# mirsadm/motioncam-decoder

Measured on AMD Instinct MI355X. Metric: MPixels/s unpacked + achieved HBM GB/s %peak, 4K 12-bit, 1/2/4/8 GPUs, higher is better.
Workload: dtype u16; 1 GPU; 3840x2160 12-bit type-7 x 240 frames/GPU, Nat (smooth field + noise sigma 12); frames_per_gpu=240, width=3840, height=2160, bits=12, encoding=7, streams=1

## Files before the change

### motioncam_decoder_amd/build.py

```python
import os
import shutil
import subprocess
import sys

PKG = os.path.dirname(os.path.abspath(__file__))
ROOT = os.path.dirname(PKG)
LIB = os.path.join(PKG, "lib")
CSRC = os.path.join(PKG, "csrc")
SYNTH = os.path.join(PKG, "synth")
HOST = os.path.join(PKG, "host")

HIPCC = os.environ.get("HIPCC") or shutil.which("hipcc") or "/opt/rocm/bin/hipcc"
ARCH = "gfx950"


def _newer(target, sources):
    if not os.path.exists(target):
        return True
    t = os.path.getmtime(target)
    return any(os.path.getmtime(s) > t for s in sources)


def _run(cmd):
    print("+", " ".join(cmd), flush=True)
    subprocess.run(cmd, check=True)


HIP_SOURCES = ("mcraw_abi.hip", "mcraw_submit.hip", "mcraw_tune.hip", "mcraw_device.hip", "mcraw_hostmem.hip", "mcraw_pool.hip",
               "mcraw_type7.hip", "mcraw_type6.hip", "mcraw_encode7.hip", "mcraw_rgb.hip", "mcraw_shade.hip")
HIP_HEADERS = ("mcraw_plan.h", "mcraw_dev.h", "mcraw_host.h", "mcraw_race.h")
HIP_FLAGS = ["--offload-arch=" + ARCH, "-O3", "-std=c++17", "-fPIC", "-fno-gpu-rdc"]


def hip_sources():
    return [os.path.join(CSRC, f) for f in HIP_SOURCES]


def _objects(flags=(), tag="", force=False, only=None):
    obj = os.path.join(LIB, "obj")
    os.makedirs(obj, exist_ok=True)
    hdrs = [os.path.join(CSRC, f) for f in HIP_HEADERS] + [os.path.join(ROOT, "include", "mcraw_hip.h")]
    objs, jobs = [], []
    for src in hip_sources():
        if only is not None and src not in only:
            continue
        o = os.path.join(obj, os.path.basename(src)[:-4] + tag + ".o")
        objs.append(o)
        if force or _newer(o, [src] + hdrs):
            cmd = [HIPCC] + HIP_FLAGS + ["-Wall", "-Wno-unused-function"] + list(flags) + ["-c", "-o", o, src]
            print("+", " ".join(cmd), flush=True)
            jobs.append((subprocess.Popen(cmd), cmd))
    for pr, cmd in jobs:
        if pr.wait() != 0:
            raise subprocess.CalledProcessError(pr.returncode, cmd)
    return objs, bool(jobs)


def _link(out, objs):
    _run([HIPCC, "--offload-arch=" + ARCH, "-shared", "-fPIC", "-fno-gpu-rdc", "-o", out] + objs + ["-lpthread"])


def build_variant(out, flags=()):
    import hashlib
    import re
    os.makedirs(os.path.dirname(os.path.abspath(out)), exist_ok=True)
    names = [re.sub(r"^-D([A-Za-z0-9_]+).*$", r"\1", f) for f in flags if f.startswith("-D")]
    everything = len(names) != len(flags) or any(n in open(os.path.join(CSRC, h)).read() for n in names for h in HIP_HEADERS)
    touched = [s for s in hip_sources() if everything or any(n in open(s).read() for n in names)]
    tag = ".v" + hashlib.sha1(" ".join(flags).encode()).hexdigest()[:10]
    plain, _ = _objects(only=[s for s in hip_sources() if s not in touched])
    special, _ = _objects(flags, tag, only=touched)
    _link(out, plain + special)
    return out


TEST_VARIANTS = (["-DMCRAW_FORCE_SEGW"], ["-DMCRAW_INJECT_MUTE7"], ["-DMCRAW_INJECT_LOST"])


def prebuild_test_variants():
    import tempfile
    with tempfile.TemporaryDirectory() as d:
        for i, flags in enumerate(TEST_VARIANTS):
            build_variant(os.path.join(d, "v%d.so" % i), flags)


def build_hip(force=False):
    os.makedirs(LIB, exist_ok=True)
    out = os.path.join(LIB, "libmcraw_hip.so")
    if os.environ.get("MCRAW_DIAG"):
        objs, built = _objects(["-DMCRAW_DIAG"], ".diag", force)
    else:
        objs, built = _objects(force=force)
    if force or built or _newer(out, objs):
        _link(out, objs)
    return out


def build_timeline(force=False):
    out = os.path.join(LIB, "timeline", "libmcraw_hip.so")
    if force or _newer(out, hip_sources() + [os.path.join(CSRC, f) for f in HIP_HEADERS]):
        build_variant(out, ["-Wall", "-Wno-unused-function", "-DMCRAW_TIMELINE"])
    return out


def build_synth(force=False):
    out = os.path.join(SYNTH, "libmcraw_synth.so")
    src = os.path.join(SYNTH, "mcraw_synth.c")
    if force or _newer(out, [src]):
        _run(["gcc", "-O3", "-march=x86-64-v3", "-fPIC", "-std=c11", "-Wall", "-Wextra", "-shared", "-o", out, src, "-lm"])
    return out


def build_host(force=False):
    os.makedirs(LIB, exist_ok=True)
    out = os.path.join(LIB, "libmotioncam_decoder.so")
    srcs = [os.path.join(HOST, f) for f in ("Decoder.cpp", "RawData.cpp", "Writer.cpp")]
    if not all(os.path.exists(s) for s in srcs):
        return None
    hdrs = [os.path.join(HOST, "include", "motioncam", f) for f in ("Decoder.hpp", "Container.hpp", "RawData.hpp", "Writer.hpp",
                                                                     "mcraw_container.h")]
    hdrs.append(os.path.join(HOST, "WorkerPool.hpp"))
    inc = ["-I" + os.path.join(HOST, "include"), "-I" + os.path.join(HOST, "thirdparty"), "-I" + os.path.join(ROOT, "include")]
    if force or _newer(out, srcs + hdrs):
        _run(["g++", "-O2", "-std=c++17", "-fPIC", "-shared", "-Wall"] + inc + ["-o", out] + srcs +
             ["-L" + LIB, "-lmcraw_hip", "-lpthread", "-Wl,-rpath,$ORIGIN"])
    tool = os.path.join(LIB, "mcraw_export")
    tsrc = os.path.join(HOST, "mcraw_export.cpp")
    if os.path.exists(tsrc) and (force or _newer(tool, [tsrc, out])):
        _run(["g++", "-O2", "-std=c++17", "-Wall"] + inc + ["-o", tool, tsrc, "-L" + LIB, "-lmotioncam_decoder",
             "-lmcraw_hip", "-lpthread", "-Wl,-rpath,$ORIGIN"])
    return out


def build_all(force=False, targets=("hip", "synth", "host")):
    res = {}
    if "hip" in targets:
        res["hip"] = build_hip(force)
    if "synth" in targets:
        res["synth"] = build_synth(force)
    if "host" in targets:
        res["host"] = build_host(force)
    return res


if __name__ == "__main__":
    if len(sys.argv) > 2 and sys.argv[1] == "variant":
        build_variant(sys.argv[2], sys.argv[3:])
        sys.exit(0)
    args = [a for a in sys.argv[1:] if not a.startswith("-")]
    build_all(force="--force" in sys.argv, targets=tuple(args) or ("hip", "synth", "host"))
```

### motioncam_decoder_amd/csrc/mcraw_type7.hip

```cpp
#include <algorithm>
#include <cstdlib>

#include "mcraw_dev.h"

#include "../../include/mcraw_hip.h"

namespace mcraw {

#define TM(p, s, n, l) ((uint32_t)((p) * 8) | ((uint32_t)(s) << 8) | ((uint32_t)((1u << (n)) - 1u) << 16) | ((uint32_t)(l) << 24))
#define Z 0u
#define ROW1(k) {TM(0, k, 1, 0), Z, Z, Z}
#define ROW2(k) {TM((k) >> 2, 2 * ((k)&3), 2, 0), Z, Z, Z}
#define ROW4(k) {TM((k) >> 1, 4 * ((k)&1), 4, 0), Z, Z, Z}
#define ROW8(k) {TM(k, 0, 8, 0), Z, Z, Z}
#define ROW10(k) {TM(5 * ((k) >> 2) + ((k)&3), 0, 8, 0), Z, Z, TM(5 * ((k) >> 2) + 4, 2 * ((k)&3), 2, 0)}
__constant__ uint32_t c_tab7[9 * 8][4] = {
    {Z, Z, Z, Z}, {Z, Z, Z, Z}, {Z, Z, Z, Z}, {Z, Z, Z, Z}, {Z, Z, Z, Z}, {Z, Z, Z, Z}, {Z, Z, Z, Z}, {Z, Z, Z, Z},
    ROW1(0), ROW1(1), ROW1(2), ROW1(3), ROW1(4), ROW1(5), ROW1(6), ROW1(7),
    ROW2(0), ROW2(1), ROW2(2), ROW2(3), ROW2(4), ROW2(5), ROW2(6), ROW2(7),
    {TM(0, 0, 3, 0), Z, Z, Z}, {TM(0, 3, 3, 0), Z, Z, Z}, {TM(0, 6, 2, 0), TM(2, 6, 1, 2), Z, Z},
    {TM(1, 0, 3, 0), Z, Z, Z}, {TM(1, 3, 3, 0), Z, Z, Z}, {TM(1, 6, 2, 0), TM(2, 7, 1, 2), Z, Z},
    {TM(2, 0, 3, 0), Z, Z, Z}, {TM(2, 3, 3, 0), Z, Z, Z},
    ROW4(0), ROW4(1), ROW4(2), ROW4(3), ROW4(4), ROW4(5), ROW4(6), ROW4(7),
    {TM(0, 0, 5, 0), Z, Z, Z}, {TM(1, 0, 5, 0), Z, Z, Z}, {TM(2, 0, 5, 0), Z, Z, Z}, {TM(3, 0, 5, 0), Z, Z, Z},
    {TM(4, 0, 5, 0), Z, Z, Z}, {TM(0, 5, 3, 0), TM(3, 5, 2, 3), Z, Z}, {TM(1, 5, 3, 0), TM(4, 5, 2, 3), Z, Z},
    {TM(2, 5, 3, 0), TM(3, 7, 1, 3), TM(4, 7, 1, 4), Z},
    {TM(0, 0, 6, 0), Z, Z, Z}, {TM(1, 0, 6, 0), Z, Z, Z}, {TM(2, 0, 6, 0), Z, Z, Z}, {TM(3, 0, 6, 0), Z, Z, Z},
    {TM(4, 0, 6, 0), Z, Z, Z}, {TM(5, 0, 6, 0), Z, Z, Z},
    {TM(0, 6, 2, 0), TM(1, 6, 2, 2), TM(2, 6, 2, 4), Z}, {TM(3, 6, 2, 0), TM(4, 6, 2, 2), TM(5, 6, 2, 4), Z},
    ROW8(0), ROW8(1), ROW8(2), ROW8(3), ROW8(4), ROW8(5), ROW8(6), ROW8(7),
    ROW10(0), ROW10(1), ROW10(2), ROW10(3), ROW10(4), ROW10(5), ROW10(6), ROW10(7),
};
#undef TM
#undef Z

__device__ __forceinline__ uint32_t term_off(uint32_t t) { return t & 0xffu; }
__device__ __forceinline__ uint32_t term_shr(uint32_t t) { return (t >> 8) & 31u; }
__device__ __forceinline__ uint32_t term_mask(uint32_t t) { return __builtin_amdgcn_perm(t, t, 0x02020202u); }
__device__ __forceinline__ uint32_t term_shl(uint32_t t) { return (t >> 24) & 31u; }

struct Unpacked { uint32_t x[4]; };

template <bool ALIGNED8>
__device__ __forceinline__ uint2 lds_read8(const uint8_t *__restrict__ base, uint32_t off)
{
    if (ALIGNED8)
        return *reinterpret_cast<const uint2 *>(base + off);
    const uint32_t *w = reinterpret_cast<const uint32_t *>(base) + (off >> 2);
    const uint32_t sh = (off & 3u) * 8u;
    const uint32_t w0 = w[0], w1 = w[1], w2 = w[2];
    return make_uint2(__builtin_amdgcn_alignbit(w1, w0, sh), __builtin_amdgcn_alignbit(w2, w1, sh));
}

template <bool ALIGNED8>
__device__ __forceinline__ Unpacked unpack8(const uint8_t *__restrict__ base, uint32_t blk, uint32_t cidx, uint32_t k,
                                            const uint4 *__restrict__ s_tab)
{
    Unpacked u;
    if (cidx >= 9u) {
        const uint2 a = lds_read8<ALIGNED8>(base, blk + 16u * k);
        const uint2 b = lds_read8<ALIGNED8>(base, blk + 16u * k + 8u);
        u.x[0] = a.x; u.x[1] = a.y; u.x[2] = b.x; u.x[3] = b.y;
        return u;
    }
    const uint4 row = s_tab[cidx * 8u + k];
    uint32_t lo = 0, hi = 0;
    const uint32_t tms[3] = {row.x, row.y, row.z};
#pragma unroll
    for (int t = 0; t < 3; t++) {
        const uint32_t tm = tms[t];
        if (!ALIGNED8 && t > 0 && !__any(tm != 0u))
            continue;
        const uint2 p = lds_read8<ALIGNED8>(base, blk + term_off(tm));
        const uint32_t m = term_mask(tm);
        lo |= ((p.x >> term_shr(tm)) & m) << term_shl(tm);
        hi |= ((p.y >> term_shr(tm)) & m) << term_shl(tm);
    }
    const uint32_t th = row.w;
    uint32_t lo8 = 0, hi8 = 0;
    if (ALIGNED8 || __any(th != 0u)) {
        const uint2 ph = lds_read8<ALIGNED8>(base, blk + term_off(th));
        const uint32_t mh = term_mask(th);
        lo8 = (ph.x >> term_shr(th)) & mh;
        hi8 = (ph.y >> term_shr(th)) & mh;
    }
    u.x[0] = __builtin_amdgcn_perm(lo8, lo, 0x05010400u);
    u.x[1] = __builtin_amdgcn_perm(lo8, lo, 0x07030602u);
    u.x[2] = __builtin_amdgcn_perm(hi8, hi, 0x05010400u);
    u.x[3] = __builtin_amdgcn_perm(hi8, hi, 0x07030602u);
    return u;
}

#ifndef MCRAW_SIDE_T
#define MCRAW_SIDE_T 512
#endif
#ifndef MCRAW_SIDE_LPT
#define MCRAW_SIDE_LPT 4
#endif
#ifndef MCRAW_SIDE_LCAP
#define MCRAW_SIDE_LCAP 512
#endif
#ifndef MCRAW_SPEC_WARM
#define MCRAW_SPEC_WARM 8192
#endif
constexpr uint32_t SIDE_XL = 9;
constexpr uint32_t SIDE_OUT = 0xFFu;
constexpr uint32_t SIDE_DEAD = 0xFEu;
static_assert(ITEM_SPLIT == 2, "k7_side sums the block lengths of half a record per item");

template <int PATTERN>
__device__ __forceinline__ uint32_t swz_xor(uint32_t v)
{
    return static_cast<uint32_t>(__builtin_amdgcn_ds_swizzle(static_cast<int>(v), PATTERN));
}

__device__ __forceinline__ void lds_barrier()
{
    asm volatile("s_waitcnt lgkmcnt(0)\n\ts_barrier" ::: "memory");
}

__device__ __forceinline__ uint2 side_strides(const uint4 v, uint32_t odd)
{
    const uint32_t pick = odd ? 0x07050301u : 0x06040200u;
    uint32_t st[2];
#pragma unroll
    for (int i = 0; i < 2; i++) {
        const uint32_t h4 = i ? __builtin_amdgcn_perm(v.w, v.z, pick) : __builtin_amdgcn_perm(v.y, v.x, pick);
        const uint32_t hb = (h4 >> 4) & 0x0F0F0F0Fu;
        const uint32_t sel = hb & 0x07070707u;
        const uint32_t lo = __builtin_amdgcn_perm(0x08060504u, 0x03020100u, sel);
        const uint32_t hi = __builtin_amdgcn_perm(0x10101010u, 0x100A0A08u, sel);
        const uint32_t g = (hb >> 3) & 0x01010101u;
        const uint32_t m = byte_mask(g);
        st[i] = (((hi & m) | (lo & ~m)) << 2) + 0x01010101u;
    }
    return make_uint2(st[0], st[1]);
}

#ifdef MCRAW_DIAG
#ifndef SIDE_PROF_BLOCK
#define SIDE_PROF_BLOCK 1u
#endif
__device__ unsigned long long g_side_prof[2][256];
#define SIDE_STAMP(slot)                                                                                               \
    do {                                                                                                               \
        if (blockIdx.x == SIDE_PROF_BLOCK && (tid == 0u || tid == 64u) && tl_n_ < 255u) {                              \
            const unsigned long long now_ = __builtin_amdgcn_s_memtime();                                              \
            g_side_prof[tid ? 1 : 0][++tl_n_] = (static_cast<unsigned long long>(slot) << 48) | (now_ - stamp_);       \
            g_side_prof[tid ? 1 : 0][0] = tl_n_;                                                                        \
        }                                                                                                              \
    } while (0)
#else
#define SIDE_STAMP(slot)
#endif

template <uint32_t SIDE_T, uint32_t SIDE_LPT, uint32_t SIDE_LCAP, uint32_t SPEC_WARM, bool PARTS, bool LASTC>
__global__ __launch_bounds__(SIDE_T) __attribute__((amdgpu_waves_per_eu(4, 4))) void k7_side(const Work7 W)
{
    constexpr uint32_t SIDE_PIECE = 16 * SIDE_T * SIDE_LPT;
    constexpr uint32_t SIDE_HALF = SIDE_PIECE / 2;
    constexpr uint32_t SIDE_BYTES = SIDE_PIECE + SIDE_XL * 16 + 16;
    __shared__ __attribute__((aligned(16))) uint8_t s_b[SIDE_BYTES];
    __shared__ __attribute__((aligned(16))) uint8_t s_T[SIDE_HALF + 80];
    __shared__ __attribute__((aligned(16))) uint16_t s_L[2][SIDE_LCAP];
    __shared__ __attribute__((aligned(16))) uint16_t s_len[2][2 * SIDE_LCAP];
    __shared__ uint4 s_tab[72];
    __shared__ __attribute__((aligned(16))) uint32_t s_st[2][4];
    __shared__ uint2 s_seg[64];
    __shared__ int32_t s_err;

    const uint32_t nfr = static_cast<uint32_t>(W.n7), nsb = PARTS ? W.nsplit[0] : 1u, nsr = PARTS ? W.nsplit[1] : 1u;
    const uint32_t bq = blockIdx.x / nfr, f = blockIdx.x - bq * nfr;
    const uint32_t s = bq < nsr ? 1u : 0u, part = s ? bq : bq - nsr, nsp = s ? nsr : nsb;
    const uint32_t fs = (nsb + nsr) * f + (s ? nsb : 0u) + part;
    const uint32_t tid = threadIdx.x, lane = tid & 63u;
    const uint32_t wave = __builtin_amdgcn_readfirstlane(tid >> 6);
#ifdef MCRAW_DIAG
    const unsigned long long stamp_ = __builtin_amdgcn_s_memtime();
    uint32_t tl_n_ = 0, nsteps_ = 0;
#endif
    if (tid < 72u)
        s_tab[tid] = reinterpret_cast<const uint4 *>(c_tab7)[tid];
    if (tid < 80u)
        s_T[SIDE_HALF + tid] = static_cast<uint8_t>(SIDE_OUT);
    if (tid == 0u)
        s_err = 0;

    const Plan7 PL = W.plans[f];
    const Plan7 *P = &PL;
    int32_t *status = W.status + fs;
    const uint32_t len = P->len;
    const __amdgpu_buffer_rsrc_t rs = frame_rsrc(P->in, len);
    SIDE_STAMP(10);

    const uint4 hv = ld_b128(rs, 0);
    const uint32_t encW = __builtin_amdgcn_readfirstlane(hv.x), encH = __builtin_amdgcn_readfirstlane(hv.y);
    const uint32_t bitsOff = __builtin_amdgcn_readfirstlane(hv.z), refsOff = __builtin_amdgcn_readfirstlane(hv.w);
    const uint32_t so = s ? refsOff : bitsOff;
    const uint64_t A0 = (static_cast<uint64_t>(so) + 4u) & ~15ull;
    const uint32_t odd = (so + 4u) & 1u;
    struct Lines {
        uint4 v[SIDE_LPT], x;
    };
    auto load_piece = [&](Lines &r, uint32_t piece) {
        const uint64_t base = A0 + static_cast<uint64_t>(piece) * SIDE_PIECE;
#pragma unroll
        for (uint32_t j = 0; j < SIDE_LPT; j++) {
            const uint64_t o = base + 16ull * (tid + SIDE_T * j);
            r.v[j] = o < len ? ld_b128(rs, static_cast<uint32_t>(o)) : make_uint4(0, 0, 0, 0);
        }
        r.x = make_uint4(0, 0, 0, 0);
        if (tid < SIDE_XL) {
            const uint64_t o = base + 16ull * (SIDE_T * SIDE_LPT + tid);
            r.x = o < len ? ld_b128(rs, static_cast<uint32_t>(o)) : make_uint4(0, 0, 0, 0);
        }
    };
    Lines nx, ny;
    load_piece(nx, 0u);
    int32_t err = 0;
    uint32_t tilesX = 0, nblk = 0, R = 0;
    if (len < 16u || bitsOff > len || refsOff > len || (encW & 63u) != 0u || encW < static_cast<uint32_t>(P->width) ||
        encW == 0u || encH == 0u || (encH & 3u) != 0u ||
        static_cast<uint64_t>(encW) * encH >= (1ull << 31)) {
        err = MCRAW_E_HEADER;
    } else {
        tilesX = encW >> 6;
        nblk = 4u * tilesX * (encH >> 2);
        R = (nblk + GROUP_BLOCKS - 1u) / GROUP_BLOCKS;
        if (R > P->ngroups)
            err = E_GEOMETRY;
        else if (so + 4u > len || so + 4u < so)
            err = MCRAW_E_TRUNCATED;
        else {
            const uint32_t count = ld_u8(rs, so) | (ld_u8(rs, so + 1u) << 8) | (ld_u8(rs, so + 2u) << 16) |
                                   (ld_u8(rs, so + 3u) << 24);
            if (__builtin_amdgcn_readfirstlane(count) < nblk)
                err = MCRAW_E_SIDESTREAM;
        }
    }
    SIDE_STAMP(11);
    Frame7 *const FR = W.frames + f;
    if (s == 0u && part == 0u && tid == 0u) {
        FR->in = P->in;
        FR->out = P->out;
        FR->len = len;
        FR->width = P->width;
        FR->rows = min(static_cast<uint32_t>(P->height), encH);
        FR->tilesX = tilesX;
        FR->nblk = err ? 0u : nblk;
        FR->fast_store = P->fast_store;
        FR->encH = encH;
        FR->pstride = P->pstride;
        for (uint32_t q = err ? 0u : nsb - 1u; q < 3u; q++) {
            FR->part_item[q] = 0xFFFFFFFFu;
            FR->part_len[q] = 0u;
        }
        W.status[W.nstatus + f] = static_cast<int32_t>(encH);
    }
    if (err) {
        if (tid == 0u)
            *status = err;
        return;
    }
    constexpr uint32_t ENDX_ = 0xFFFFFFFFu;
    uint32_t m_lo = 0u, m_hi = 0xFFFFFFFFu, np_guess = 0xFFFFFFFFu;
    if (nsp > 1u) {
        const uint32_t other = s ? bitsOff : refsOff;
        const uint64_t end_guess = other > so ? other : len;
        const uint64_t npieces = (end_guess - A0 + SIDE_PIECE - 1u) / SIDE_PIECE;
        np_guess = static_cast<uint32_t>(npieces);
        m_lo = static_cast<uint32_t>(part * npieces / nsp);
        if (part + 1u < nsp)
            m_hi = static_cast<uint32_t>((part + 1u) * npieces / nsp);
    }
    uint64_t *const sync = W.sync + (static_cast<size_t>(2u * f + s) * MAX_SPLIT7 + part) * 2u;
    uint16_t *const rp_base = (PARTS && nsp > 1u && W.rpos) ? W.rpos + (static_cast<size_t>(2u * f + s) * MAX_SPLIT7 + part) * W.Rmax : nullptr;
    const __amdgpu_buffer_rsrc_t rsp = frame_rsrc(reinterpret_cast<const uint8_t *>(rp_base), rp_base ? 2u * W.Rmax : 0u);
    uint32_t rleft = 0u, rnext = 0u, rexit = ENDX_;
    bool rdead = false;
    constexpr uint32_t ENDX = ENDX_;

    uint8_t *bits = W.bits + static_cast<size_t>(f) * W.Rmax * 64u;
    uint16_t *refs = W.refs + static_cast<size_t>(f) * W.Rmax * 64u;
    uint32_t *goff = W.grp_off + static_cast<size_t>(f) * (W.Rmax * ITEM_SPLIT + 1u);

    uint32_t upc = 0;
    uint32_t bb = 0;
    uint32_t tb = 0;
    uint32_t n = 0;
    uint64_t carry = 0u;
    uint32_t n_first = 0xFFFFFFFFu;
    int32_t lane_err = 0;
    bool dead = false;
    uint32_t decode_from = 0u;
    constexpr uint32_t NOENTRY = 0xFFFFFFFEu;
    static_assert(SPEC_WARM <= SIDE_HALF, "a speculative count starts inside the piece in front of the part's first");

    auto store_bytes = [&](const Lines &r) {
#pragma unroll
        for (uint32_t j = 0; j < SIDE_LPT; j++)
            reinterpret_cast<uint4 *>(s_b)[tid + SIDE_T * j] = r.v[j];
        if (tid < SIDE_XL)
            reinterpret_cast<uint4 *>(s_b)[SIDE_T * SIDE_LPT + tid] = r.x;
    };
    auto build_strides = [&](const Lines &r, uint32_t piece) {
        const uint64_t base = A0 + static_cast<uint64_t>(piece) * SIDE_PIECE;
        const uint64_t left = len - min(static_cast<uint64_t>(len), base);
        const uint32_t lim = static_cast<uint32_t>(min(left, static_cast<uint64_t>(1u << 30)));
#pragma unroll
        for (uint32_t j = 0; j < SIDE_LPT; j++) {
            const uint32_t line = tid + SIDE_T * j;
            uint2 st = side_strides(r.v[j], odd);
            if (16u * line + 16u + 130u > lim) {
                uint32_t w[2] = {st.x, st.y};
#pragma unroll
                for (uint32_t i = 0; i < 8u; i++) {
                    const uint32_t sv = (w[i >> 2] >> (8u * (i & 3u))) & 0xffu;
                    if (16u * line + 2u * i + odd + 2u * sv > lim)
                        w[i >> 2] = (w[i >> 2] & ~(0xffu << (8u * (i & 3u)))) | (SIDE_DEAD << (8u * (i & 3u)));
                }
                st = make_uint2(w[0], w[1]);
            }
            reinterpret_cast<uint2 *>(s_T)[line] = st;
        }
    };
    #ifndef MCRAW_SEGW_RATIO
#define MCRAW_SEGW_RATIO 3u
#endif
#ifndef MCRAW_WARM_SEGS
#define MCRAW_WARM_SEGS 4
#endif
    constexpr uint32_t SEG_C = SIDE_HALF / 64u, WARM_C = MCRAW_WARM_SEGS * SEG_C, SEG_NONE = 0x7FFFu, SEG_DEADX = 0xFFFFu;
#ifdef MCRAW_FORCE_SEGW
    bool segw = true, seg_valid = false;
#else
    bool segw = false, seg_valid = false;
#endif
    uint32_t seg_total = 0, seg_done = 0, seg_exit = 0;
    auto seg_chain = [&](bool on, uint32_t pos, uint32_t segs, uint32_t sege, uint32_t &ent, uint32_t &cnt, uint32_t &ex) {
        pos = on ? pos : SIDE_HALF;
        sege = on ? sege : 0u;
        bool stop;
        do {
#pragma unroll
            for (int u = 0; u < 2; u++) {
                const uint32_t code = s_T[pos];
                stop = pos >= sege || code >= SIDE_DEAD;
                const bool inseg = !stop && pos >= segs;
                ent = min(ent, inseg ? pos : SEG_NONE);
                cnt += inseg ? 1u : 0u;
                pos += stop ? 0u : code;
            }
#ifdef MCRAW_DIAG
            nsteps_ += 2;
#endif
        } while (__any(!stop));
        if (on)
            ex = pos >= sege ? pos : SEG_DEADX;
    };
    auto seg_walk = [&](uint32_t org) {
        const uint32_t segs = org + lane * SEG_C;
        const bool act = segs < SIDE_HALF;
        const uint32_t sege = min(segs + SEG_C, SIDE_HALF);
        const bool on_chain = lane < WARM_C / SEG_C;
        uint32_t ent = SEG_NONE, cnt = 0, ex = SEG_DEADX;
        seg_chain(act, on_chain ? org : segs - WARM_C, segs, sege, ent, cnt, ex);
        uint32_t src = SEG_NONE;
        for (uint32_t round = 0; round < 64u; round++) {
            const uint32_t want = wave_prev(ex, ex);
            const uint32_t claim = src != SEG_NONE ? src : ent != SEG_NONE ? ent : ex;
            const bool bad = act && !on_chain && claim != want;
            if (__ballot(bad) == 0ull)
                break;
            if (bad) {
                ent = SEG_NONE;
                cnt = 0;
                ex = SEG_DEADX;
                src = want;
            }
            seg_chain(bad && want != SEG_DEADX, want, segs, sege, ent, cnt, ex);
        }
        uint32_t total;
        const uint32_t off = wave_excl_scan(act ? cnt : 0u, lane, &total);
        s_seg[lane] = make_uint2((ent & 0xFFFFu) | (cnt << 16), off);
        const uint32_t nact = (SIDE_HALF - org + SEG_C - 1u) / SEG_C;
        seg_exit = static_cast<uint32_t>(__builtin_amdgcn_readlane(static_cast<int>(ex), static_cast<int>(min(nact, 64u) - 1u)));
        seg_total = total;
        seg_done = 0;
        seg_valid = true;
    };
    auto seg_list = [&](uint16_t *L, uint32_t take) {
        const uint2 sv = s_seg[lane];
        const uint32_t cnt = sv.x >> 16, off = sv.y, lo = seg_done, hi = seg_done + take;
        uint32_t pos = sv.x & 0xFFFFu, kk = off;
        const uint32_t kend = min(off + cnt, hi);
        bool part = cnt != 0u && off < hi && off + cnt > lo;
        pos = part ? pos : SIDE_HALF;
        while (__any(part)) {
            const uint32_t code = s_T[pos];
            if (part && kk >= lo)
                L[kk - lo] = static_cast<uint16_t>(pos);
            kk++;
            part = part && kk < kend;
            pos = part ? pos + code : SIDE_HALF;
        }
    };
    auto walk = [&](uint32_t lst, uint32_t pu, uint32_t SU, uint32_t room, bool fresh) {
        uint16_t *L = s_L[lst];
        uint32_t cnt = 0, why = 2u;
        if (!segw && pu < SIDE_HALF) {
            uint32_t nb, take, nxt, passes = 0;
            bool go;
            do {
                const uint32_t u = pu + lane * SU;
                const uint32_t code = s_T[min(u, SIDE_HALF)];
                const unsigned long long m = __ballot(code != SU);
                nb = m == 0ull ? 64u : static_cast<uint32_t>(__builtin_ctzll(m));
                take = min(nb, room - cnt);
                if (lane < take)
                    L[cnt + lane] = static_cast<uint16_t>(u);
                nxt = static_cast<uint32_t>(__builtin_amdgcn_readlane(static_cast<int>(code), static_cast<int>(nb & 63u)));
                cnt += take;
                pu += take * SU;
                go = take == nb && cnt < room && (nb == 64u || nxt < SIDE_DEAD);
                SU = (go && nb != 64u) ? nxt : SU;
                passes++;
                segw = go && passes >= 8u && passes * MCRAW_SEGW_RATIO > cnt;
#ifdef MCRAW_DIAG
                nsteps_++;
#endif
            } while (go && !segw);
            if (segw) {
            } else if (take < nb) {
                why = 1u;
            } else if (cnt >= room) {
                why = 1u;
                SU = (nb != 64u && nxt < SIDE_DEAD) ? nxt : 0u;
            } else {
                why = nxt == SIDE_OUT ? 2u : 3u;
                SU = 0u;
            }
            if (segw)
                seg_valid = false;
        } else if (!segw) {
            SU = 0u;
        }
        if (segw && pu < SIDE_HALF) {
            if (fresh || !seg_valid)
                seg_walk(pu);
            const uint32_t take = min(room - cnt, seg_total - seg_done);
            if (take)
                seg_list(L + cnt, take);
            seg_done += take;
            cnt += take;
            SU = 0u;
            if (seg_done == seg_total) {
                why = seg_exit == SEG_DEADX ? 3u : 2u;
                pu = seg_exit == SEG_DEADX ? 0u : seg_exit;
                seg_valid = false;
            } else {
                why = 1u;
                pu = 0u;
            }
        } else if (segw) {
            SU = 0u;
        }
        if (lane == 0u)
            *reinterpret_cast<uint4 *>(s_st[lst]) = make_uint4(pu, cnt, why, SU);
    };

    const uint32_t k = lane & 7u, sub = lane >> 3;
    const uint32_t first_cand = static_cast<uint32_t>((so + 4u) & 15u) >> 1;
    static_assert((2u * SIDE_LCAP) % 512u == 0u, "whole passes of 512 items");
    auto scan_unit = [&](uint32_t par, uint32_t n0, uint32_t cnt) {
        const uint32_t nitems = 2u * cnt;
        for (uint32_t base = 0; base < nitems; base += 512u) {
            const uint32_t i0 = base + 8u * lane;
            uint4 lv = make_uint4(0u, 0u, 0u, 0u);
            if (i0 < nitems)
                lv = *reinterpret_cast<const uint4 *>(&s_len[par][i0]);
            uint32_t a[8] = {lv.x & 0xffffu, lv.x >> 16, lv.y & 0xffffu, lv.y >> 16,
                             lv.z & 0xffffu, lv.z >> 16, lv.w & 0xffffu, lv.w >> 16};
            uint32_t mine = 0;
#pragma unroll
            for (uint32_t i = 0; i < 8u; i++) {
                a[i] = i0 + i < nitems ? a[i] : 0u;
                mine += a[i];
            }
            uint32_t utot;
            const uint32_t ex = wave_excl_scan(mine, lane, &utot);
            uint32_t o = static_cast<uint32_t>(carry) + ex;
#pragma unroll
            for (uint32_t i = 0; i < 8u; i++) {
                if (i0 + i < nitems)
                    goff[2u * n0 + i0 + i] = o;
                o += a[i];
            }
            carry += utot;
        }
    };

#ifdef MCRAW_INJECT_MUTE7
    constexpr uint32_t SPIN7 = 1u << 6;
#else
    constexpr uint32_t SPIN7 = 1u << 19;
#endif
    __shared__ uint32_t s_ask[4];
    bool told = part + 1u >= nsp;
    auto tell = [&](uint32_t count, uint32_t where) {
        if (!told && tid == 0u) {
#ifdef MCRAW_INJECT_MUTE7
            if (part != 0u)
#endif
            {
                look_put(sync, W.epoch, count);
                look_put(sync + 1, W.epoch, where);
            }
        }
        told = true;
    };
    auto ask = [&](uint32_t &count, uint32_t &where) {
        lds_barrier();
        if (tid == 0u) {
            uint32_t c = 0u, w = first_cand, ok = 1u;
            if (part) {
                ok = 0u;
                for (uint32_t spin = 0; spin < SPIN7; spin++) {
                    if (look_get(sync - 2, W.epoch, &c) && look_get(sync - 1, W.epoch, &w)) {
                        ok = 1u;
                        break;
                    }
                    __builtin_amdgcn_s_sleep(8);
                }
            }
            s_ask[0] = c;
            s_ask[1] = w;
            s_ask[2] = ok;
        }
        lds_barrier();
        count = s_ask[0];
        where = s_ask[1];
        return s_ask[2] != 0u;
    };
    auto nothing_to_decode = [&]() {
        if (tid == 0u && s == 0u && nsp > 1u) {
            if (part + 1u < nsp)
                FR->part_len[part] = 0u;
            if (part)
                FR->part_item[part - 1u] = 0xFFFFFFFFu;
        }
    };

    uint32_t run_piece = 0u, run_cand = first_cand, run_n = 0u;
    uint32_t nx_piece = 0u;
    uint32_t exitc = ENDX;
    bool go = true;
    if (nsp > 1u) {
        const bool empty = m_lo >= m_hi, lastp = part + 1u >= nsp;
        const bool owns0 = !empty && m_lo == 0u;
        const uint32_t m_chi = lastp ? np_guess : m_hi;
        const bool lastc = LASTC && lastp && !owns0 && rp_base != nullptr && m_chi > m_lo && m_chi != 0xFFFFFFFFu;
        const bool spec = !empty && !owns0 && (!lastp || lastc);
        uint32_t entry = NOENTRY, cnt1 = 0u, exit1 = ENDX;
        bool dead1 = false;
        bool counted = false;
        if (!empty && (!lastp || lastc)) {
            counted = true;
            uint32_t spiece = 0xFFFFFFFFu;
            uint32_t cpiece = spec ? m_lo - 1u : 0u, lst = 0u;
            if (spec)
                load_piece(nx, cpiece);
            build_strides(nx, cpiece);
            load_piece(nx, cpiece + 1u);
            nx_piece = cpiece + 1u;
            lds_barrier();
            if (wave == 0u)
                walk(0u, spec ? SIDE_HALF - SPEC_WARM : first_cand, 0u, spec ? SIDE_LCAP : min(R, SIDE_LCAP), true);
            for (;;) {
                lds_barrier();
                const uint4 st4 = *reinterpret_cast<const uint4 *>(s_st[lst]);
                const uint32_t pu = __builtin_amdgcn_readfirstlane(st4.x);
                const uint32_t total = __builtin_amdgcn_readfirstlane(st4.y);
                const uint32_t why = __builtin_amdgcn_readfirstlane(st4.z);
                const uint32_t SU = __builtin_amdgcn_readfirstlane(st4.w);
                const uint32_t npc = why == 2u ? cpiece + 1u : cpiece;
                if (cpiece >= m_lo) {
                    if (rp_base && total) {
                        const uint16_t *Lc = s_L[lst];
                        for (uint32_t i = tid; i < total; i += SIDE_T)
                            if (cnt1 + i < W.Rmax)
                                rp_base[cnt1 + i] = static_cast<uint16_t>(Lc[i] | ((i == 0u && cpiece != spiece) ? 0x8000u : 0u));
                        spiece = cpiece;
                    }
                    cnt1 += total;
                    dead1 = dead1 || why == 3u;
                }
// ... 33 lines not shown
        uint32_t pn = 0u, pw = first_cand;
        const bool ok = owns0 ? true : ask(pn, pw);
        SIDE_STAMP(21);
        decode_from = m_lo;
        if (!ok) {
            if (empty) {
                decode_from = 0xFFFFFFFFu;
                if (m_hi == 0u) {
                    tell(0u, first_cand);
                    nothing_to_decode();
                    go = false;
                }
            }
        } else if (!owns0 && (pw == ENDX || pn >= R)) {
            tell(pn, ENDX);
            nothing_to_decode();
            go = false;
        } else if (empty) {
            tell(pn, pw);
            nothing_to_decode();
            go = false;
        } else if (lastp) {
            run_piece = m_lo, run_cand = owns0 ? first_cand : pw, run_n = pn;
            if (lastc && pw == entry)
                replay_from_count();
        } else if (owns0 || pw == entry) {
            const uint32_t upto = pn + cnt1;
            tell(min(upto, R), upto >= R || dead1 || exit1 == ENDX ? ENDX : exit1);
            run_piece = m_lo, run_cand = owns0 ? first_cand : entry, run_n = pn;
            replay_from_count();
        } else {
            run_piece = m_lo, run_cand = pw, run_n = pn;
        }
        if (go && run_n >= R) {
            tell(run_n, ENDX);
            nothing_to_decode();
            go = false;
        }
    }

    uint32_t cur = 0;
    uint32_t prev_n = 0, prev_total = 0;
    if (go) {
    lds_barrier();
    upc = bb = tb = run_piece;
    n = run_n;
#ifdef MCRAW_FORCE_SEGW
    segw = true;
#else
    segw = false;
#endif
    seg_valid = false;
    carry = run_piece == 0u && decode_from == 0u ? 16u : 0u;
    if (nx_piece != run_piece)
        load_piece(nx, run_piece);
    store_bytes(nx);
    SIDE_STAMP(12);
    if (!rleft)
        build_strides(nx, run_piece);
    load_piece(nx, run_piece + 1u);
    load_piece(ny, run_piece + 2u);
    uint4 rq = make_uint4(0u, 0u, 0u, 0u);
    auto rfetch = [&](uint32_t at) { rq = ld_b128_nt(rsp, 2u * (at + 8u * lane)); };
    auto replay = [&](uint32_t lst, uint32_t room) {
        const uint32_t n = min(room, rleft);
        const uint32_t w4[4] = {rq.x, rq.y, rq.z, rq.w};
        uint32_t mine = 8u, ment = 0u;
#pragma unroll
        for (int i = 7; i >= 0; i--) {
            const uint32_t idx = 8u * lane + static_cast<uint32_t>(i), e = (w4[i >> 1] >> (16 * (i & 1))) & 0xffffu;
            const bool hit = idx >= 1u && idx < n && (e & 0x8000u) != 0u;
            mine = hit ? static_cast<uint32_t>(i) : mine;
            ment = hit ? e : ment;
        }
        const unsigned long long m = __ballot(mine != 8u);
        uint32_t take = n, pu = 0u, why = 1u;
        if (m) {
            const uint32_t fl = static_cast<uint32_t>(__builtin_ctzll(m));
            take = 8u * fl + wave_lane(mine, fl);
            pu = SIDE_HALF + (wave_lane(ment, fl) & 0x7fffu);
            why = 2u;
        } else if (n == rleft) {
            if (rdead)
                why = 3u;
            else if (rexit != ENDX)
                why = 2u, pu = SIDE_HALF + rexit;
        }
        if (8u * lane < take)
            *reinterpret_cast<uint4 *>(&s_L[lst][8u * lane]) = make_uint4(rq.x & 0x7fff7fffu, rq.y & 0x7fff7fffu, rq.z & 0x7fff7fffu, rq.w & 0x7fff7fffu);
        if (lane == 0u)
            *reinterpret_cast<uint4 *>(s_st[lst]) = make_uint4(pu, take, why, 0u);
        rfetch(rnext + take);
    };
    lds_barrier();
    SIDE_STAMP(13);
    if (wave == 0u) {
        if (rleft) {
            rfetch(0u);
            replay(0u, min(R - run_n, SIDE_LCAP / 4u));
        } else
            walk(0u, run_cand, 0u, min(R - run_n, SIDE_LCAP / 4u), true);
    }
    SIDE_STAMP(14);
    while (true) {
        lds_barrier();
        SIDE_STAMP(0);
        const uint4 st4 = *reinterpret_cast<const uint4 *>(s_st[cur]);
        const uint32_t pu = __builtin_amdgcn_readfirstlane(st4.x);
        const uint32_t total = __builtin_amdgcn_readfirstlane(st4.y);
        const uint32_t why = __builtin_amdgcn_readfirstlane(st4.z);
        const uint32_t SU = __builtin_amdgcn_readfirstlane(st4.w);
        const uint32_t npc = why == 2u ? upc + 1u : upc;
        const bool last = n + total >= R || why == 3u || npc >= m_hi;
        const bool skip = upc < decode_from;
        if (!skip && n_first == 0xFFFFFFFFu)
            n_first = n;
        if (npc > upc && npc == m_hi)
            exitc = pu - SIDE_HALF;
        if (rleft) {
            rleft -= min(total, rleft);
            rnext += total;
        }
        const bool moved = upc > bb, build = !last && npc > tb && rleft == 0u;
        if (moved) {
            store_bytes(nx);
            bb = upc;
            nx = ny;
            load_piece(ny, bb + 2u);
        }
        if (build) {
            build_strides(nx, npc);
            tb = npc;
        }
        if (moved || build)
            lds_barrier();
        SIDE_STAMP(1);
        if (wave == 0u) {
            if (!last) {
                if (rleft)
                    replay(cur ^ 1u, min(R - (n + total), SIDE_LCAP));
                else
                    walk(cur ^ 1u, npc > upc ? pu - SIDE_HALF : pu, SU, min(R - (n + total), SIDE_LCAP), npc > upc);
            }
            SIDE_STAMP(2);
            if (s == 0u && prev_total)
                scan_unit(cur ^ 1u, prev_n, prev_total);
            SIDE_STAMP(5);
        } else if (!skip) {
            const uint8_t *B = s_b;
            const uint16_t *L = s_L[cur];
            constexpr uint32_t STEP = (SIDE_T / 64u - 1u) * 8u;
            uint32_t q = (wave - 1u) * 8u + sub;
            uint32_t ro_n = q < total ? 2u * L[q] + odd : 0u;
            uint32_t hd_n = *reinterpret_cast<const uint16_t *>(B + (ro_n & ~1u)) | (static_cast<uint32_t>(B[(ro_n & ~1u) + 2u]) << 16);
            for (uint32_t qb = (wave - 1u) * 8u; qb < total; qb += STEP, q += STEP) {
                const bool live = q < total;
                const uint32_t ro = ro_n;
                const uint32_t hd = hd_n >> (8u * (ro & 1u));
                ro_n = q + STEP < total ? 2u * L[q + STEP] + odd : 0u;
                hd_n = *reinterpret_cast<const uint16_t *>(B + (ro_n & ~1u)) | (static_cast<uint32_t>(B[(ro_n & ~1u) + 2u]) << 16);
                const uint32_t b0 = live ? hd & 0xffu : 0u, b1 = (hd >> 8) & 0xffu;
                const uint32_t hb = b0 >> 4, ref = ((b0 & 15u) << 8) | b1;
                Unpacked U = unpack8<false>(B, ro + 2u, cls7_of(hb), k, s_tab);
                const u16x2 rr = __builtin_bit_cast(u16x2, ref | (ref << 16));
#pragma unroll
                for (int i = 0; i < 4; i++)
                    U.x[i] = __builtin_bit_cast(uint32_t, __builtin_bit_cast(u16x2, U.x[i]) + rr);
                const uint32_t r = n + q;
                const uint32_t idx = r * 64u + 8u * k;
                if (s == 1u) {
                    if (live)
                        *reinterpret_cast<uint4 *>(refs + idx) = make_uint4(U.x[0], U.x[1], U.x[2], U.x[3]);
                    continue;
                }
                const uint32_t nvalid = live ? min(8u, nblk - min(nblk, idx)) : 0u;
                if (nvalid < 8u) {
#pragma unroll
                    for (uint32_t i = 0; i < 4u; i++)
                        U.x[i] &= nvalid >= 2u * i + 2u ? 0xffffffffu : nvalid == 2u * i + 1u ? 0xffffu : 0u;
                }
                uint32_t c[4], over = 0;
#pragma unroll
                for (uint32_t i = 0; i < 4u; i++) {
                    c[i] = __builtin_bit_cast(uint32_t, __builtin_elementwise_min(__builtin_bit_cast(u16x2, U.x[i]),
                                                                                  __builtin_bit_cast(u16x2, 0x00100010u)));
                    over |= c[i] ^ U.x[i];
                }
                if (over)
                    lane_err |= MCRAW_E_SIDESTREAM;
                const uint32_t bytes_lo = __builtin_amdgcn_perm(c[1], c[0], 0x06040200u);
                const uint32_t bytes_hi = __builtin_amdgcn_perm(c[3], c[2], 0x06040200u);
                if (live)
                    *reinterpret_cast<uint2 *>(bits + idx) = make_uint2(bytes_lo, bytes_hi);
                uint32_t l8 = 0;
#pragma unroll
                for (uint32_t i = 0; i < 2u; i++) {
                    const uint32_t v4 = i ? bytes_hi : bytes_lo;
                    const uint32_t sel = v4 & 0x07070707u;
                    const uint32_t lo = __builtin_amdgcn_perm(0x08060504u, 0x03020100u, sel);
                    const uint32_t hi = __builtin_amdgcn_perm(0x10101010u, 0x100A0A08u, sel);
                    const uint32_t g = (v4 >> 3) & 0x01010101u;
                    const uint32_t m = byte_mask(g);
                    const uint32_t l4 = ((hi & m) | (lo & ~m)) | (v4 & 0x10101010u);
                    l8 = __builtin_amdgcn_sad_u8(l4, 0u, l8);
                }
                l8 += swz_xor<0x041F>(l8);
                l8 += swz_xor<0x081F>(l8);
                if (live && (k & 3u) == 0u)
                    s_len[cur][2u * q + (k >> 2)] = static_cast<uint16_t>(l8 << 3);
            }
            SIDE_STAMP(3);
        }
        prev_n = n;
        prev_total = skip ? 0u : total;
        n += total;
        if (last) {
            dead = why == 3u && n < R && !skip;
            break;
        }
        upc = npc;
        cur ^= 1u;
    }
    tell(min(n, R), n >= R || dead || exitc == ENDX ? ENDX : exitc);
    if (s == 0u && prev_total) {
        lds_barrier();
        if (wave == 0u)
            scan_unit(cur, prev_n, prev_total);
    }
    if (tid == 0u) {
        if (dead)
            lane_err |= MCRAW_E_TRUNCATED;
        if (s == 0u) {
            const uint32_t c32 = static_cast<uint32_t>(min(carry, static_cast<uint64_t>(0xffffffffu)));
            if (n >= R && !dead && n_first != 0xFFFFFFFFu) {
                goff[ITEM_SPLIT * R] = c32;
                if (nsp == 1u && carry > len)
                    lane_err |= MCRAW_E_TRUNCATED;
            }
            if (nsp > 1u) {
                if (part + 1u < nsp)
                    FR->part_len[part] = n_first != 0xFFFFFFFFu ? c32 : 0u;
                if (part)
                    FR->part_item[part - 1u] = n_first != 0xFFFFFFFFu ? ITEM_SPLIT * n_first : 0xFFFFFFFFu;
            }
        }
    }
    }
    if (lane_err)
        atomicOr(&s_err, lane_err);
    lds_barrier();
    if (tid == 0u)
        *status = s_err;
    SIDE_STAMP(15);
#ifdef MCRAW_DIAG
    if (blockIdx.x == SIDE_PROF_BLOCK && tid == 0u)
        g_side_prof[0][255] = nsteps_;
#endif
}

constexpr int PAY_LDS = ITEM_SPAN + 16 + 32;
constexpr uint32_t PAY_CHUNKS = ITEM_SPAN / 16 + 1;

struct ItemS {
    uint32_t valid;
    uint32_t g, nblk, tilesX;
    uint32_t base16, n16, head;
    int32_t width, rows;
    uint32_t fast;
    const uint8_t *in;
    uint32_t len;
    uint16_t *out;
    size_t meta;
    uint32_t lean;
    uint32_t pstride;
};

__device__ __forceinline__ ItemS item_scalars(const Work7 &W, uint32_t item, uint32_t first_frame, uint32_t class_groups)
{
    ItemS I;
    const uint32_t per = W.Rmax * ITEM_SPLIT;
    const uint32_t cper = class_groups * ITEM_SPLIT;
    const uint32_t fc = item / cper;
    const uint32_t f = first_frame + fc;
    const uint32_t g = item - fc * cper;
    const Frame7 *F = W.frames + f;
    const uint32_t nblk = F->nblk;
    const uint32_t *grp = W.grp_off + static_cast<size_t>(f) * (per + 1u) + g;
    I.valid = g * ITEM_BLOCKS < nblk ? 1u : 0u;
    uint32_t start = 0, end = 0;
    if (I.valid) {
        start = grp[0];
        end = grp[1];
        if (W.nsplit[0] > 1u) {
            uint32_t ps = 0u, pe = 0u, sum_s = 0u;
            uint64_t e64 = end;
#pragma unroll
            for (uint32_t q = 0; q < 3u; q++) {
                const uint32_t pi = F->part_item[q];
                ps = g >= pi ? q + 1u : ps;
                pe = g + 1u >= pi && pi != 0xFFFFFFFFu ? q + 1u : pe;
            }
#pragma unroll
            for (uint32_t q = 0; q < 3u; q++) {
                const uint32_t pl = F->part_len[q];
                sum_s += q < ps ? pl : 0u;
                e64 += q < pe ? pl : 0u;
            }
            start += sum_s;
            end = static_cast<uint32_t>(e64);
            if ((g + 1u) * ITEM_BLOCKS >= nblk && e64 > F->len)
                atomicOr(W.status + (W.nsplit[0] + W.nsplit[1]) * f, MCRAW_E_TRUNCATED);
        }
    }
    I.g = g;
    I.nblk = nblk;
    I.tilesX = F->tilesX;
    I.base16 = start & ~15u;
    I.head = start - I.base16;
    I.n16 = I.valid ? min((end - min(end, I.base16) + 15u) >> 4, PAY_CHUNKS) : 0u;
    I.width = F->width;
    I.rows = static_cast<int32_t>(F->rows);
    I.fast = F->fast_store;
    I.in = F->in;
    I.len = F->len;
    I.out = F->out;
    I.meta = static_cast<size_t>(f) * W.Rmax * 64u + static_cast<size_t>(g) * ITEM_BLOCKS;
    I.lean = 0u;
    I.pstride = F->pstride;
    return I;
}

template <bool NT = false, int POST = 0>
__device__ __forceinline__ void store_px8(const ItemS &I, const Post &post, uint32_t y, uint32_t x, uint32_t p[4])
{
    const uint32_t width = static_cast<uint32_t>(I.width);
    if (y >= static_cast<uint32_t>(I.rows) || x >= width)
        return;
    if constexpr (POST >= PK_F32) {
        float_store8<NT, POST>(I.out, post, post.inv, width, I.pstride, y, x, p, min(8u, width - x), I.fast != 0u);
        return;
    } else if (POST) {
        post_store8<NT, POST>(I.out, post, width, y, x, p, min(8u, width - x), I.fast != 0u, POST != 16 && I.lean != 0u);
        return;
    }
    uint16_t *dst = I.out + static_cast<size_t>(y) * static_cast<size_t>(width) + x;
    if (I.fast && x + 8u <= width) {
        typedef uint32_t u32x4 __attribute__((ext_vector_type(4)));
        const u32x4 v = {p[0], p[1], p[2], p[3]};
        if (NT)
            store_stream16(dst, v);
        else
            *gptr<u32x4>(dst) = v;
    } else if (x + 8u <= width) {
        typedef uint32_t u32x4_u __attribute__((ext_vector_type(4), aligned(2)));
        const u32x4_u v = {p[0], p[1], p[2], p[3]};
        *gptr<u32x4_u>(dst) = v;
    } else {
        const uint32_t n = width - x;
#pragma unroll
        for (uint32_t i = 0; i < 8u; i++)
// ... 213 lines not shown
```

Before: 1.980 million MPixels/s.

## Add wave-uniform class fast paths to type-7 side decode and restructure run scan

In the side-stream decode loop, when all lanes of a wave share one block class, the code now uses specialised unpack routines per class. For small classes in the bit pass it computes the output bytes directly and skips the generic clamp and pack. The run-scan loop is reorganised into groups of four ballot steps with raised wave priority, the L index is prefetched two steps ahead, and the ds_swizzle reductions are replaced by DPP quad permutes. A compile flag keeps the old generic path as a test variant. The cost is extra branches, ballots and code size.

```diff
diff --git a/motioncam_decoder_amd/build.py b/motioncam_decoder_amd/build.py
--- a/motioncam_decoder_amd/build.py
+++ b/motioncam_decoder_amd/build.py
@@ -74,7 +74,7 @@
     return out
 
 
-TEST_VARIANTS = (["-DMCRAW_FORCE_SEGW"], ["-DMCRAW_INJECT_MUTE7"], ["-DMCRAW_INJECT_LOST"])
+TEST_VARIANTS = (["-DMCRAW_FORCE_SEGW"], ["-DMCRAW_INJECT_MUTE7"], ["-DMCRAW_INJECT_LOST"], ["-DMCRAW_SIDE_GENERIC"])
 
 
 def prebuild_test_variants():
diff --git a/motioncam_decoder_amd/csrc/mcraw_type7.hip b/motioncam_decoder_amd/csrc/mcraw_type7.hip
--- a/motioncam_decoder_amd/csrc/mcraw_type7.hip
+++ b/motioncam_decoder_amd/csrc/mcraw_type7.hip
@@ -91,6 +91,61 @@
     return u;
 }
 
+struct __attribute__((packed, aligned(1))) PackedU2 { uint32_t x, y; };
+__device__ __forceinline__ uint2 lds_read8_any(const uint8_t *__restrict__ base, uint32_t off)
+{
+#ifdef MCRAW_SIDE_READ64
+    const PackedU2 v = *reinterpret_cast<const PackedU2 *>(base + off);
+    return make_uint2(v.x, v.y);
+#else
+    return lds_read8<false>(base, off);
+#endif
+}
+
+template <uint32_t CLS>
+__device__ __forceinline__ uint2 side_bytes_class(const uint8_t *__restrict__ base, uint32_t blk, uint32_t k)
+{
+    static_assert(CLS == 1u || CLS == 2u || CLS == 4u || CLS == 7u, "classes of one term");
+    constexpr uint32_t LOG = CLS == 1u ? 0u : CLS == 2u ? 1u : CLS == 4u ? 2u : 3u, N = 1u << LOG;
+    constexpr uint32_t MASK = ((1u << N) - 1u) * 0x01010101u;
+    const uint2 p = lds_read8_any(base, blk + 8u * (k >> (3u - LOG)));
+    if (LOG == 3u)
+        return p;
+    const uint32_t sh = (k & ((8u >> LOG) - 1u)) << LOG;
+    return make_uint2((p.x >> sh) & MASK, (p.y >> sh) & MASK);
+}
+
+template <uint32_t CLS>
+__device__ __forceinline__ Unpacked side_unpack_class(const uint8_t *__restrict__ base, uint32_t blk, uint32_t k)
+{
+    Unpacked u;
+    if (CLS == 0u) {
+        u.x[0] = u.x[1] = u.x[2] = u.x[3] = 0u;
+        return u;
+    }
+    if (CLS == 9u) {
+        const uint2 a = lds_read8_any(base, blk + 16u * k);
+        const uint2 b = lds_read8_any(base, blk + 16u * k + 8u);
+        u.x[0] = a.x; u.x[1] = a.y; u.x[2] = b.x; u.x[3] = b.y;
+        return u;
+    }
+    uint2 lo, hi8 = make_uint2(0u, 0u);
+    if (CLS == 8u) {
+        const uint32_t g = 40u * (k >> 2);
+        lo = lds_read8_any(base, blk + g + 8u * (k & 3u));
+        const uint2 ph = lds_read8_any(base, blk + g + 32u);
+        const uint32_t sh = 2u * (k & 3u);
+        hi8 = make_uint2((ph.x >> sh) & 0x03030303u, (ph.y >> sh) & 0x03030303u);
+    } else {
+        lo = side_bytes_class<(CLS == 1u || CLS == 2u || CLS == 4u) ? CLS : 7u>(base, blk, k);
+    }
+    u.x[0] = __builtin_amdgcn_perm(hi8.x, lo.x, 0x05010400u);
+    u.x[1] = __builtin_amdgcn_perm(hi8.x, lo.x, 0x07030602u);
+    u.x[2] = __builtin_amdgcn_perm(hi8.y, lo.y, 0x05010400u);
+    u.x[3] = __builtin_amdgcn_perm(hi8.y, lo.y, 0x07030602u);
+    return u;
+}
+
 #ifndef MCRAW_SIDE_T
 #define MCRAW_SIDE_T 512
 #endif
@@ -108,10 +163,10 @@
 constexpr uint32_t SIDE_DEAD = 0xFEu;
 static_assert(ITEM_SPLIT == 2, "k7_side sums the block lengths of half a record per item");
 
-template <int PATTERN>
-__device__ __forceinline__ uint32_t swz_xor(uint32_t v)
-{
-    return static_cast<uint32_t>(__builtin_amdgcn_ds_swizzle(static_cast<int>(v), PATTERN));
+template <int CTRL>
+__device__ __forceinline__ uint32_t quad_perm(uint32_t v)
+{
+    return static_cast<uint32_t>(__builtin_amdgcn_update_dpp(0, static_cast<int>(v), CTRL, 0xf, 0xf, true));
 }
 
 __device__ __forceinline__ void lds_barrier()
@@ -409,39 +464,58 @@
         uint16_t *L = s_L[lst];
         uint32_t cnt = 0, why = 2u;
         if (!segw && pu < SIDE_HALF) {
-            uint32_t nb, take, nxt, passes = 0;
-            bool go;
-            do {
-                const uint32_t u = pu + lane * SU;
-                const uint32_t code = s_T[min(u, SIDE_HALF)];
-                const unsigned long long m = __ballot(code != SU);
-                nb = m == 0ull ? 64u : static_cast<uint32_t>(__builtin_ctzll(m));
-                take = min(nb, room - cnt);
-                if (lane < take)
-                    L[cnt + lane] = static_cast<uint16_t>(u);
-                nxt = static_cast<uint32_t>(__builtin_amdgcn_readlane(static_cast<int>(code), static_cast<int>(nb & 63u)));
-                cnt += take;
-                pu += take * SU;
-                go = take == nb && cnt < room && (nb == 64u || nxt < SIDE_DEAD);
-                SU = (go && nb != 64u) ? nxt : SU;
-                passes++;
-                segw = go && passes >= 8u && passes * MCRAW_SEGW_RATIO > cnt;
+            __builtin_amdgcn_s_setprio(3);
+            uint32_t nb, take, nxt, lim, left = room, passes = 0, SUp = SU;
+            for (;;) {
+                uint32_t i = 4u;
+                bool more;
+                do {
+                    const uint32_t u = __umul24(lane, SU) + pu;
+                    const uint32_t code = s_T[min(u, SIDE_HALF)];
+                    const unsigned long long m = __ballot(code != SU);
+                    nb = m == 0ull ? 64u : static_cast<uint32_t>(__builtin_ctzll(m));
+                    take = min(nb, left);
+                    if (lane < take)
+                        L[cnt + lane] = static_cast<uint16_t>(u);
+                    nxt = static_cast<uint32_t>(__builtin_amdgcn_readlane(static_cast<int>(code), static_cast<int>(nb & 63u)));
+                    cnt += take;
+                    pu += take * SU;
 #ifdef MCRAW_DIAG
-                nsteps_++;
-#endif
-            } while (go && !segw);
+                    nsteps_++;
+#endif
+                    lim = nxt < SIDE_DEAD ? left : 0u;
+                    asm volatile("" : "+s"(lim));
+                    i--;
+                    uint32_t lim4 = min(lim, i << 16);
+                    asm volatile("" : "+s"(lim4));
+                    more = nb < lim4;
+                    left -= take;
+                    SUp = SU;
+                    SU = nxt;
+                } while (more);
+                if (nb >= lim) {
+                    left += take;
+                    SU = SUp;
+                    break;
+                }
+                passes += 4u;
+                if (passes >= 8u && passes * MCRAW_SEGW_RATIO > cnt) {
+                    segw = true;
+                    break;
+                }
+            }
+            __builtin_amdgcn_s_setprio(0);
             if (segw) {
+                seg_valid = false;
             } else if (take < nb) {
                 why = 1u;
-            } else if (cnt >= room) {
+            } else if (take == left) {
                 why = 1u;
                 SU = (nb != 64u && nxt < SIDE_DEAD) ? nxt : 0u;
             } else {
                 why = nxt == SIDE_OUT ? 2u : 3u;
                 SU = 0u;
             }
-            if (segw)
-                seg_valid = false;
         } else if (!segw) {
             SU = 0u;
         }
@@ -781,44 +855,86 @@
             constexpr uint32_t STEP = (SIDE_T / 64u - 1u) * 8u;
             uint32_t q = (wave - 1u) * 8u + sub;
             uint32_t ro_n = q < total ? 2u * L[q] + odd : 0u;
+            uint32_t ro_nn = q + STEP < total ? 2u * L[q + STEP] + odd : 0u;
             uint32_t hd_n = *reinterpret_cast<const uint16_t *>(B + (ro_n & ~1u)) | (static_cast<uint32_t>(B[(ro_n & ~1u) + 2u]) << 16);
             for (uint32_t qb = (wave - 1u) * 8u; qb < total; qb += STEP, q += STEP) {
                 const bool live = q < total;
                 const uint32_t ro = ro_n;
                 const uint32_t hd = hd_n >> (8u * (ro & 1u));
-                ro_n = q + STEP < total ? 2u * L[q + STEP] + odd : 0u;
+                ro_n = ro_nn;
                 hd_n = *reinterpret_cast<const uint16_t *>(B + (ro_n & ~1u)) | (static_cast<uint32_t>(B[(ro_n & ~1u) + 2u]) << 16);
+                const uint32_t l_nn = L[min(q + 2u * STEP, SIDE_LCAP - 1u)];
                 const uint32_t b0 = live ? hd & 0xffu : 0u, b1 = (hd >> 8) & 0xffu;
                 const uint32_t hb = b0 >> 4, ref = ((b0 & 15u) << 8) | b1;
-                Unpacked U = unpack8<false>(B, ro + 2u, cls7_of(hb), k, s_tab);
-                const u16x2 rr = __builtin_bit_cast(u16x2, ref | (ref << 16));
-#pragma unroll
-                for (int i = 0; i < 4; i++)
-                    U.x[i] = __builtin_bit_cast(uint32_t, __builtin_bit_cast(u16x2, U.x[i]) + rr);
+                const uint32_t cls = cls7_of(hb);
                 const uint32_t r = n + q;
                 const uint32_t idx = r * 64u + 8u * k;
+                Unpacked U;
+                uint32_t bytes_lo = 0u, bytes_hi = 0u;
+                uint32_t path = 0u;
+#ifndef MCRAW_SIDE_GENERIC
+                if (qb + 8u <= total) {
+                    const uint32_t c0 = __builtin_amdgcn_readfirstlane(cls);
+                    if (__ballot(cls != c0) == 0ull) {
+                        if (s == 1u) {
+                            path = 1u;
+                            switch (c0) {
+                            case 0u: U = side_unpack_class<0u>(B, ro + 2u, k); break;
+                            case 7u: U = side_unpack_class<7u>(B, ro + 2u, k); break;
+                            case 8u: U = side_unpack_class<8u>(B, ro + 2u, k); break;
+                            case 9u: U = side_unpack_class<9u>(B, ro + 2u, k); break;
+                            default: path = 0u; break;
+                            }
+                        } else if (c0 <= 2u && (n + qb + 8u) * 64u <= nblk) {
+                            const uint32_t top = 16u - ((1u << c0) - 1u);
+                            if (__ballot(ref > top) == 0ull) {
+                                path = 2u;
+                                uint2 p = make_uint2(0u, 0u);
+                                if (c0 == 1u)
+                                    p = side_bytes_class<1u>(B, ro + 2u, k);
+                                else if (c0 == 2u)
+                                    p = side_bytes_class<2u>(B, ro + 2u, k);
+                                const uint32_t refb = __builtin_amdgcn_perm(ref, ref, 0u);
+                                bytes_lo = p.x + refb;
+                                bytes_hi = p.y + refb;
+                            }
+                        }
+                    }
+                }
+#endif
+                if (path == 0u)
+                    U = unpack8<false>(B, ro + 2u, cls, k, s_tab);
+                ro_nn = (2u * l_nn + odd) & (2u * SIDE_HALF - 1u);
+                if (path != 2u) {
+                    const u16x2 rr = __builtin_bit_cast(u16x2, ref | (ref << 16));
+#pragma unroll
+                    for (int i = 0; i < 4; i++)
+                        U.x[i] = __builtin_bit_cast(uint32_t, __builtin_bit_cast(u16x2, U.x[i]) + rr);
+                }
                 if (s == 1u) {
                     if (live)
                         *reinterpret_cast<uint4 *>(refs + idx) = make_uint4(U.x[0], U.x[1], U.x[2], U.x[3]);
                     continue;
                 }
-                const uint32_t nvalid = live ? min(8u, nblk - min(nblk, idx)) : 0u;
-                if (nvalid < 8u) {
-#pragma unroll
-                    for (uint32_t i = 0; i < 4u; i++)
-                        U.x[i] &= nvalid >= 2u * i + 2u ? 0xffffffffu : nvalid == 2u * i + 1u ? 0xffffu : 0u;
+                if (path != 2u) {
+                    const uint32_t nvalid = live ? min(8u, nblk - min(nblk, idx)) : 0u;
+                    if (nvalid < 8u) {
+#pragma unroll
+                        for (uint32_t i = 0; i < 4u; i++)
+                            U.x[i] &= nvalid >= 2u * i + 2u ? 0xffffffffu : nvalid == 2u * i + 1u ? 0xffffu : 0u;
+                    }
+                    uint32_t c[4], over = 0;
+#pragma unroll
+                    for (uint32_t i = 0; i < 4u; i++) {
+                        c[i] = __builtin_bit_cast(uint32_t, __builtin_elementwise_min(__builtin_bit_cast(u16x2, U.x[i]),
+                                                                                      __builtin_bit_cast(u16x2, 0x00100010u)));
+                        over |= c[i] ^ U.x[i];
+                    }
+                    if (over)
+                        lane_err |= MCRAW_E_SIDESTREAM;
+                    bytes_lo = __builtin_amdgcn_perm(c[1], c[0], 0x06040200u);
+                    bytes_hi = __builtin_amdgcn_perm(c[3], c[2], 0x06040200u);
                 }
-                uint32_t c[4], over = 0;
-#pragma unroll
-                for (uint32_t i = 0; i < 4u; i++) {
-                    c[i] = __builtin_bit_cast(uint32_t, __builtin_elementwise_min(__builtin_bit_cast(u16x2, U.x[i]),
-                                                                                  __builtin_bit_cast(u16x2, 0x00100010u)));
-                    over |= c[i] ^ U.x[i];
-                }
-                if (over)
-                    lane_err |= MCRAW_E_SIDESTREAM;
-                const uint32_t bytes_lo = __builtin_amdgcn_perm(c[1], c[0], 0x06040200u);
-                const uint32_t bytes_hi = __builtin_amdgcn_perm(c[3], c[2], 0x06040200u);
                 if (live)
                     *reinterpret_cast<uint2 *>(bits + idx) = make_uint2(bytes_lo, bytes_hi);
                 uint32_t l8 = 0;
@@ -833,8 +949,8 @@
                     const uint32_t l4 = ((hi & m) | (lo & ~m)) | (v4 & 0x10101010u);
                     l8 = __builtin_amdgcn_sad_u8(l4, 0u, l8);
                 }
-                l8 += swz_xor<0x041F>(l8);
-                l8 += swz_xor<0x081F>(l8);
+                l8 += quad_perm<0xB1>(l8);
+                l8 += quad_perm<0x4E>(l8);
                 if (live && (k & 3u) == 0u)
                     s_len[cur][2u * q + (k >> 2)] = static_cast<uint16_t>(l8 << 3);
             }
```

Result: no change. 1.974 million MPixels/s (-0.3%).
